# MikeWangWZHL/VidIL

Hardware: AMD Instinct MI355X
Metric: frames/sec whole-node (BLIP caption+filt + CLIP visual-token) 224^2 8f/video (higher is better)
Workload: dtype bf16

## Files before the change

vidil_amd/csrc/attention.hip:

```cpp
#include <type_traits>

#include "common.h"
#include "gemm_epilogue.h"

namespace {

template <typename T>
struct AttnP {
  const T* q;
  const T* k;
  const T* vt;
  T* out;
  const int32_t* kv_len;
  const int32_t* kv_index;
  const int32_t* group_start;
  int Bq, H, Nq, Nk, Tq_cap, Tk_cap, NP, kv_group, causal, causal_off, ldo, n_kv;
  int out_mode;
  int tiled;
  int rb;
  int ostage;
  const float* q32;
  long long ldq32;
  float q_scale;
};
// ... 94 lines not shown
#pragma unroll
  for (int r = 0; r < 16; ++r) {
    const float e = __builtin_amdgcn_exp2f(__builtin_fmaf(S[r], kLog2e, -mc));
    S[r] = e;
    ps += e;
  }
  l = FIRST ? ps : l + ps;
#pragma unroll
  for (int hb = 0; hb < 2; ++hb)
#pragma unroll
    for (int j = 0; j < 8; ++j) pf[hb][j] = (T)S[hb * 8 + j];
}

template <typename T, bool MASKED = true, bool LAZY = true, bool FIRST = false, typename VFrag>
__device__ __forceinline__ void softmax_pv_tile(f32x16& S, int key0, int klim, bool need_mask, float& m, float& l,
                                                f32x16 (&O)[2], VFrag&& vfrag) {
  typename Elt<T>::x8 pf[2];
  softmax_tile<T, MASKED, FIRST, LAZY>(S, key0, klim, need_mask, m, l, O, pf);
#pragma unroll
  for (int hb = 0; hb < 2; ++hb) {
#pragma unroll
    for (int dt = 0; dt < 2; ++dt) {
      const typename Elt<T>::x8 vf = vfrag(dt, hb);
      O[dt] = Elt<T>::mfma32(vf, pf[hb], O[dt]);
    }
  }
}

template <typename T, typename VFrag>
__device__ __forceinline__ void softmax_pv_tile_psplit(f32x16& S, int key0, int klim, bool need_mask, float& m, float& l,
                                                       f32x16 (&O)[2], VFrag&& vfrag) {
  const int hi = (threadIdx.x & 63) >> 5;
  if (need_mask) {
#pragma unroll
    for (int r = 0; r < 16; ++r) {
      const int key = key0 + (r & 3) + 8 * (r >> 2) + 4 * hi;
      if (key >= klim) S[r] = -INFINITY;
    }
  }
  float mt = S[0];
#pragma unroll
  for (int r = 1; r < 16; ++r) mt = fmaxf(mt, S[r]);
  mt = fmaxf(mt, __shfl_xor(mt, 32, 64));
  const float mn = fmaxf(m, mt);
  const float mc = (mn == -INFINITY ? 0.f : mn) * kLog2e;
  const float alpha = __builtin_amdgcn_exp2f(__builtin_fmaf(m, kLog2e, -mc));
  l *= alpha;
  m = mn;
#pragma unroll
  for (int dt = 0; dt < 2; ++dt)
#pragma unroll
    for (int r = 0; r < 16; ++r) O[dt][r] *= alpha;
  typename Elt<T>::x8 ph[2], pl[2];
  float ps = 0.f;
#pragma unroll
  for (int r = 0; r < 16; ++r) {
    const float e = __builtin_amdgcn_exp2f(__builtin_fmaf(S[r], kLog2e, -mc));
    ps += e;
    const T eh = Elt<T>::from_f32(e);
    ph[r >> 3][r & 7] = eh;
    pl[r >> 3][r & 7] = Elt<T>::from_f32(e - (float)eh);
  }
  l += ps;
#pragma unroll
  for (int hb = 0; hb < 2; ++hb) {
#pragma unroll
    for (int dt = 0; dt < 2; ++dt) {
      const typename Elt<T>::x8 vf = vfrag(dt, hb);
      O[dt] = Elt<T>::mfma32(vf, pl[hb], O[dt]);
      O[dt] = Elt<T>::mfma32(vf, ph[hb], O[dt]);
    }
  }
}

template <typename T>
__device__ __forceinline__ void store_rows(const AttnP<T>& p, const RowInfo& ri, int h, const f32x16 (&O)[2], float inv) {
  using f16x4 = typename Elt<T>::x4;
  using f16 = T;
  if (!ri.valid) return;
  const int hi = (threadIdx.x & 63) >> 5;
  if (p.out_mode >= 2) {
    const int pl = p.ldo / 3;
    f16* og = p.out + ((size_t)ri.qb * p.Nq + ri.t) * p.ldo + h * 64 + 4 * hi;
#pragma unroll
    for (int dt = 0; dt < 2; ++dt)
#pragma unroll
      for (int rq = 0; rq < 4; ++rq) {
        f16x4 vh, vl;
#pragma unroll
        for (int e = 0; e < 4; ++e) {
          const float v = O[dt][rq * 4 + e] * inv;
          vh[e] = Elt<T>::from_f32(v);
          vl[e] = Elt<T>::from_f32(v - (float)vh[e]);
        }
        *(f16x4*)(og + dt * 32 + rq * 8) = vh;
        *(f16x4*)(og + pl + dt * 32 + rq * 8) = vl;
        if (p.out_mode == 2) *(f16x4*)(og + 2 * pl + dt * 32 + rq * 8) = vh;
      }
    return;
  }
  if (p.out_mode == 1) {
    uint8_t* o8 = (uint8_t*)p.out + ((size_t)ri.qb * p.Nq + ri.t) * p.ldo + h * 64 + 4 * hi;
#pragma unroll
    for (int dt = 0; dt < 2; ++dt)
#pragma unroll
      for (int rq = 0; rq < 4; ++rq)
        *(uint32_t*)(o8 + dt * 32 + rq * 8) = pack4_fp8(O[dt][rq * 4 + 0] * inv, O[dt][rq * 4 + 1] * inv, O[dt][rq * 4 + 2] * inv,
                                                        O[dt][rq * 4 + 3] * inv);
    return;
  }
  f16* og = p.out + ((size_t)ri.qb * p.Nq + ri.t) * p.ldo + h * 64 + 4 * hi;
#pragma unroll
  for (int dt = 0; dt < 2; ++dt)
#pragma unroll
    for (int rq = 0; rq < 4; ++rq) {
      const f16x4 v = {(f16)(O[dt][rq * 4 + 0] * inv), (f16)(O[dt][rq * 4 + 1] * inv), (f16)(O[dt][rq * 4 + 2] * inv),
                       (f16)(O[dt][rq * 4 + 3] * inv)};
      *(f16x4*)(og + dt * 32 + rq * 8) = v;
    }
}

template <typename T>
__device__ __forceinline__ void store_rows_lds(const AttnP<T>& p, const RowInfo& ri, int h, const f32x16 (&O)[2], float inv, char* scratch) {
  using f16 = T;
  using f16x4 = typename Elt<T>::x4;
  using f16x8 = typename Elt<T>::x8;
  const int lane = threadIdx.x & 63;
  const int hi = lane >> 5, l31 = lane & 31;
  const long long own = ri.valid ? (long long)(((size_t)ri.qb * p.Nq + ri.t) * p.ldo + h * 64) : -1;
  long long dst[2];
#pragma unroll
  for (int i = 0; i < 2; ++i) {
    const int r = i * 16 + (lane >> 2);
    const int lo = __shfl((int)(own & 0xffffffffLL), r, 64), hi32 = __shfl((int)(own >> 32), r, 64);
    dst[i] = ((long long)hi32 << 32) | (unsigned int)lo;
  }
#pragma unroll
  for (int dt = 0; dt < 2; ++dt) {
#pragma unroll
    for (int rq = 0; rq < 4; ++rq) {
      const f16x4 v = {(f16)(O[dt][rq * 4 + 0] * inv), (f16)(O[dt][rq * 4 + 1] * inv), (f16)(O[dt][rq * 4 + 2] * inv),
                       (f16)(O[dt][rq * 4 + 3] * inv)};
      *(f16x4*)(scratch + l31 * 64 + ((rq ^ ((l31 >> 1) & 3)) << 4) + hi * 8) = v;
    }
#pragma unroll
    for (int i = 0; i < 2; ++i) {
      const int r = i * 16 + (lane >> 2), c = lane & 3;
      const f16x8 v = *(const f16x8*)(scratch + r * 64 + ((c ^ ((r >> 1) & 3)) << 4));
      if (dst[i] >= 0) *(f16x8*)(p.out + dst[i] + dt * 32 + c * 8) = v;
    }
  }
}

template <typename T, int NKT, int NW>
__global__ __launch_bounds__(NW * 64, NW == 8 ? 4 : 2) void attn_lds_kernel(const AttnP<T> p) {
  using f16 = T;
  using f16x8 = typename Elt<T>::x8;
  constexpr int NKEY = NKT * 32;
  constexpr int VROW = NKEY + 8;
  constexpr int NT = NW * 64;
  extern __shared__ __attribute__((aligned(16))) char smem[];
  f16* Ks = (f16*)smem;
  f16* Vs = (f16*)(smem + NKEY * KROW * 2);

  const int tid = threadIdx.x;
  const int lane = tid & 63;
  const int wave = __builtin_amdgcn_readfirstlane(tid >> 6);
  const int hi = lane >> 5, l31 = lane & 31;
  const int h = blockIdx.y;
  int bk, first, count;
  resolve_unit(p, blockIdx.z, bk, first, count);
  const int rows = count * p.Nq;
  const int nk = p.Nk;
  const int rows_per_wg = NW * 32 * (nk <= NKEY ? p.rb : 1);
  const int base = blockIdx.x * rows_per_wg;
  if (base >= rows) return;

  const f16* kg = p.k + ((size_t)bk * p.H + h) * p.Tk_cap * 64;
  const f16* vg = p.vt + ((size_t)bk * p.H + h) * 64 * (size_t)p.NP;
  constexpr int KIT = (NKEY * 8 + NT - 1) / NT;
  constexpr int VIT = (64 * NKT * 4 + NT - 1) / NT;
  auto stage = [&](int k0) {
    f16x8 kreg[KIT], vreg[VIT];
#pragma unroll
    for (int i = 0; i < KIT; ++i) {
      const int q = tid + i * NT;
      const int row = q >> 3, c = q & 7;
      kreg[i] = zero8<T>();
      if (q < NKEY * 8 && k0 + row < nk) kreg[i] = *(const f16x8*)(kg + (size_t)(k0 + row) * 64 + c * 8);
    }
    if (p.NP == 0) {
      const f16* vrow = p.vt + ((size_t)bk * p.H + h) * p.Tk_cap * 64;
#pragma unroll
      for (int i = 0; i < KIT; ++i) {
        const int q = tid + i * NT;
        const int c = q / NKEY, r = q - c * NKEY;
        vreg[i] = zero8<T>();
        if (q < NKEY * 8 && k0 + r < nk) vreg[i] = *(const f16x8*)(vrow + (size_t)(k0 + r) * 64 + c * 8);
      }
    } else {
#pragma unroll
      for (int i = 0; i < VIT; ++i) {
        const int q = tid + i * NT;
        const int d = q / (NKT * 4), kc = q - d * (NKT * 4);
        const int pos0 = k0 + kc * 8;
        vreg[i] = zero8<T>();
        if (q < 64 * NKT * 4 && (pos0 & ~15) < nk && pos0 + 8 <= p.NP) vreg[i] = *(const f16x8*)(vg + (size_t)d * p.NP + pos0);
      }
    }
#pragma unroll
    for (int i = 0; i < KIT; ++i) {
      const int q = tid + i * NT;
      if (q < NKEY * 8) *(f16x8*)(Ks + (q >> 3) * KROW + (q & 7) * 8) = kreg[i];
    }
    if (p.NP == 0) {
#pragma unroll
      for (int i = 0; i < KIT; ++i) {
        const int q = tid + i * NT;
        const int c = q / NKEY, r = q - c * NKEY;
        if (q < NKEY * 8) {
          const int col = vt_pos(r);
#pragma unroll
          for (int e = 0; e < 8; ++e) Vs[(c * 8 + e) * VROW + col] = vreg[i][e];
        }
      }
    } else {
#pragma unroll
      for (int i = 0; i < VIT; ++i) {
        const int q = tid + i * NT;
        const int d = q / (NKT * 4), kc = q - d * (NKT * 4);
        const int pos0 = k0 + kc * 8;
        if (q < 64 * NKT * 4) {
          f16x8 v = vreg[i];
          if ((pos0 | 15) + 1 > nk) {
#pragma unroll
            for (int e = 0; e < 8; ++e)
              if (vt_pos(pos0 + e) >= nk) v[e] = (f16)0.f;
          }
          *(f16x8*)(Vs + d * VROW + kc * 8) = v;
        }
      }
    }
  };

  auto stage_next = [&](int k0) {
    for (int q = tid; q < NKEY * 8; q += NT) {
      const int row = q >> 3, c = q & 7;
      f16x8 v = zero8<T>();
      if (k0 + row < nk) v = *(const f16x8*)(kg + (size_t)(k0 + row) * 64 + c * 8);
      *(f16x8*)(Ks + row * KROW + c * 8) = v;
    }
    if (p.NP == 0) {
      const f16* vrow = p.vt + ((size_t)bk * p.H + h) * p.Tk_cap * 64;
      for (int q = tid; q < NKEY * 8; q += NT) {
        const int c = q / NKEY, r = q - c * NKEY;
        f16x8 v = zero8<T>();
        if (k0 + r < nk) v = *(const f16x8*)(vrow + (size_t)(k0 + r) * 64 + c * 8);
        const int col = vt_pos(r);
#pragma unroll
        for (int e = 0; e < 8; ++e) Vs[(c * 8 + e) * VROW + col] = v[e];
      }
    }
    for (int q = tid; p.NP != 0 && q < 64 * NKT * 4; q += NT) {
      const int d = q / (NKT * 4), kc = q - d * (NKT * 4);
      const int pos0 = k0 + kc * 8;
      const int blk_end = (pos0 | 15) + 1;
      f16x8 v = zero8<T>();
      if (blk_end <= nk) {
        v = *(const f16x8*)(vg + (size_t)d * p.NP + pos0);
      } else if ((pos0 & ~15) < nk && pos0 + 8 <= p.NP) {
        v = *(const f16x8*)(vg + (size_t)d * p.NP + pos0);
#pragma unroll
        for (int e = 0; e < 8; ++e)
          if (vt_pos(pos0 + e) >= nk) v[e] = (f16)0.f;
      }
      *(f16x8*)(Vs + d * VROW + kc * 8) = v;
    }
  };

  const int nblk = nk <= NKEY ? p.rb : 1;
  RowInfo ri;
  f16x8 qf[4];
  bool active;
  auto load_q = [&](int rbi) {
    const int v0 = base + (rbi * NW + wave) * 32;
    active = v0 < rows;
    ri = row_info(p, (active ? v0 : 0) + l31, first, rows);
    const f16* qg = p.q + (((size_t)ri.qb * p.H + h) * p.Tq_cap + ri.t) * 64 + hi * 8;
#pragma unroll
    for (int ks = 0; ks < 4; ++ks) qf[ks] = *(const f16x8*)(qg + ks * 16);
  };
  load_q(0);
  stage(0);
  __syncthreads();
#pragma unroll 1
  for (int rbi = 0; rbi < nblk; ++rbi) {
    if (rbi > 0) {
      load_q(rbi);
      if (!active) break;
    }
    int kmin = ri.klim;
#pragma unroll
    for (int o = 32; o > 0; o >>= 1) {
      const int x = __shfl_xor(kmin, o, 64);
      kmin = x < kmin ? x : kmin;
    }

    float m = -INFINITY, l = 0.f;
    f32x16 O[2];
#pragma unroll
    for (int dt = 0; dt < 2; ++dt)
#pragma unroll
      for (int r = 0; r < 16; ++r) O[dt][r] = 0.f;

#pragma unroll 1
    for (int k0 = 0; k0 < nk; k0 += NKEY) {
      if (rbi == 0 && k0 > 0) {
        __syncthreads();
        stage_next(k0);
        __syncthreads();
      }
      if (!active) continue;

#pragma unroll 1
      for (int kt = 0; kt < NKT; ++kt) {
        if (k0 + kt * 32 >= nk) break;
        f32x16 S;
#pragma unroll
        for (int r = 0; r < 16; ++r) S[r] = 0.f;
#pragma unroll
        for (int ks = 0; ks < 4; ++ks) {
          const f16x8 kf = *(const f16x8*)(Ks + (kt * 32 + l31) * KROW + ks * 16 + hi * 8);
          S = Elt<T>::mfma32(kf, qf[ks], S);
        }
        const bool need_mask = (k0 + kt * 32 + 32) > kmin;
        auto vfrag = [&](int dt, int hb) { return *(const f16x8*)(Vs + (dt * 32 + l31) * VROW + (kt * 2 + hb) * 16 + 8 * hi); };
        if (need_mask) softmax_pv_tile<T, true>(S, k0 + kt * 32, ri.klim, true, m, l, O, vfrag);
        else softmax_pv_tile<T, false>(S, k0 + kt * 32, ri.klim, false, m, l, O, vfrag);
      }
    }
    if (!active) break;
    l += __shfl_xor(l, 32, 64);
    if (p.out_mode == 0 && p.ostage)
      store_rows_lds(p, ri, h, O, l > 0.f ? 1.0f / l : 0.f, smem + NKEY * KROW * 2 + 64 * VROW * 2 + wave * 2048);
    else
      store_rows(p, ri, h, O, l > 0.f ? 1.0f / l : 0.f);
  }
}

constexpr int LONG_NKT = 4;
constexpr int LONG_NKEY = LONG_NKT * 32;
constexpr int kLongMaxNk = 16384;

template <typename T, int NW>
__global__ __launch_bounds__(NW * 64, NW == 8 ? 4 : 2) void attn_long_kernel(const AttnP<T> p) {
  using f16 = T;
  using f16x8 = typename Elt<T>::x8;
  constexpr int NKT = LONG_NKT, NKEY = LONG_NKEY;
  constexpr int VROW = NKEY + 8;
  constexpr int NT = NW * 64;
  constexpr int BUF = NKEY * KROW * 2 + 64 * VROW * 2;
  constexpr int KIT = NKEY * 8 / NT;
  static_assert(NKEY * 8 % NT == 0 && 64 * NKT * 4 == NKEY * 8, "a chunk is a whole number of pieces per thread");
  extern __shared__ __attribute__((aligned(16))) char smem[];

  const int tid = threadIdx.x;
  const int lane = tid & 63;
  const int wave = __builtin_amdgcn_readfirstlane(tid >> 6);
  const int hi = lane >> 5, l31 = lane & 31;
  const int h = blockIdx.y;
  int bk, first, count;
  resolve_unit(p, blockIdx.z, bk, first, count);
  const int rows = count * p.Nq;
  const int nk = p.Nk;
  const int base = blockIdx.x * (NW * 32);
  if (base >= rows) return;

  const f16* kg = p.k + ((size_t)bk * p.H + h) * p.Tk_cap * 64;
  const f16* vg = p.vt + ((size_t)bk * p.H + h) * 64 * (size_t)p.NP;
  const f16* vrow = p.vt + ((size_t)bk * p.H + h) * p.Tk_cap * 64;
  const bool vrm = p.NP == 0;

  f16x8 kreg[KIT], vreg[KIT];
  const __amdgpu_buffer_rsrc_t rk = uniform_rsrc(kg, (uint32_t)nk * 128u);
  const __amdgpu_buffer_rsrc_t rv = vrm ? uniform_rsrc(vrow, (uint32_t)nk * 128u) : uniform_rsrc(vg, 128u * (uint32_t)p.NP);
  auto gload = [&](int k0) {
#pragma unroll
    for (int i = 0; i < KIT; ++i) {
      const int q = tid + i * NT;
      kreg[i] = __builtin_bit_cast(f16x8, __builtin_amdgcn_raw_buffer_load_b128(rk, (k0 * 8 + q) * 16, 0, 0));
    }
    if (vrm) {
#pragma unroll
      for (int i = 0; i < KIT; ++i) {
        const int q = tid + i * NT;
        const int c = q / NKEY, r = q - c * NKEY;
        vreg[i] = __builtin_bit_cast(f16x8, __builtin_amdgcn_raw_buffer_load_b128(rv, (k0 + r) * 128 + c * 16, 0, 0));
      }
    } else {
#pragma unroll
      for (int i = 0; i < KIT; ++i) {
        const int q = tid + i * NT;
        const int d = q / (NKT * 4), kc = q - d * (NKT * 4);
        const int pos0 = k0 + kc * 8;
        const bool in = (pos0 & ~15) < nk && pos0 + 8 <= p.NP;
        vreg[i] = __builtin_bit_cast(f16x8, __builtin_amdgcn_raw_buffer_load_b128(rv, in ? (d * p.NP + pos0) * 2 : (int)0x80000000, 0, 0));
      }
    }
  };
  auto lstore = [&](int k0, char* buf) {
    f16* Ks = (f16*)buf;
    f16* Vs = (f16*)(buf + NKEY * KROW * 2);
#pragma unroll
    for (int i = 0; i < KIT; ++i) {
      const int q = tid + i * NT;
      *(f16x8*)(Ks + (q >> 3) * KROW + (q & 7) * 8) = kreg[i];
    }
    if (vrm) {
#pragma unroll
      for (int i = 0; i < KIT; ++i) {
        const int q = tid + i * NT;
        const int c = q / NKEY, r = q - c * NKEY;
        const int col = vt_pos(r);
#pragma unroll
        for (int e = 0; e < 8; ++e) Vs[(c * 8 + e) * VROW + col] = vreg[i][e];
      }
    } else {
#pragma unroll
      for (int i = 0; i < KIT; ++i) {
        const int q = tid + i * NT;
        const int d = q / (NKT * 4), kc = q - d * (NKT * 4);
        const int pos0 = k0 + kc * 8;
        f16x8 v = vreg[i];
        if ((pos0 | 15) + 1 > nk) {
#pragma unroll
          for (int e = 0; e < 8; ++e)
            if (vt_pos(pos0 + e) >= nk) v[e] = (f16)0.f;
        }
        *(f16x8*)(Vs + d * VROW + kc * 8) = v;
      }
    }
  };

  const int v0 = base + wave * 32;
  const bool active = v0 < rows;
  const RowInfo ri = row_info(p, (active ? v0 : 0) + l31, first, rows);
  f16x8 qf[4];
  {
    const f16* qg = p.q + (((size_t)ri.qb * p.H + h) * p.Tq_cap + ri.t) * 64 + hi * 8;
#pragma unroll
    for (int ks = 0; ks < 4; ++ks) qf[ks] = *(const f16x8*)(qg + ks * 16);
  }
  gload(0);
  int kmin = ri.klim, kmax = ri.klim;
#pragma unroll
  for (int o = 32; o > 0; o >>= 1) {
    const int x = __shfl_xor(kmin, o, 64), y = __shfl_xor(kmax, o, 64);
    kmin = x < kmin ? x : kmin;
    kmax = y > kmax ? y : kmax;
  }
  float m = -INFINITY, l = 0.f;
  f32x16 O[2];
#pragma unroll
  for (int dt = 0; dt < 2; ++dt)
#pragma unroll
    for (int r = 0; r < 16; ++r) O[dt][r] = 0.f;

  lstore(0, smem);
  if (NKEY < nk) gload(NKEY);
  __syncthreads();
  int cur = 0;
#pragma unroll 1
  for (int k0 = 0; k0 < nk; k0 += NKEY) {
    if (active) {
      const f16* Ks = (const f16*)(smem + cur * BUF);
      const f16* Vs = (const f16*)(smem + cur * BUF + NKEY * KROW * 2);
#pragma unroll 1
      for (int kt = 0; kt < NKT; ++kt) {
        const int key0 = k0 + kt * 32;
        if (key0 >= nk || key0 >= kmax) break;
        f32x16 S;
#pragma unroll
        for (int r = 0; r < 16; ++r) S[r] = 0.f;
#pragma unroll
        for (int ks = 0; ks < 4; ++ks) {
          const f16x8 kf = *(const f16x8*)(Ks + (kt * 32 + l31) * KROW + ks * 16 + hi * 8);
          S = Elt<T>::mfma32(kf, qf[ks], S);
        }
        const bool need_mask = (key0 + 32) > kmin;
        auto vfrag = [&](int dt, int hb) { return *(const f16x8*)(Vs + (dt * 32 + l31) * VROW + (kt * 2 + hb) * 16 + 8 * hi); };
        if (need_mask) softmax_pv_tile<T, true>(S, key0, ri.klim, true, m, l, O, vfrag);
        else softmax_pv_tile<T, false>(S, key0, ri.klim, false, m, l, O, vfrag);
      }
    }
    if (k0 + NKEY < nk) {
      lstore(k0 + NKEY, smem + (cur ^ 1) * BUF);
      if (k0 + 2 * NKEY < nk) gload(k0 + 2 * NKEY);
    }
    __syncthreads();
    cur ^= 1;
  }
  if (!active) return;
  l += __shfl_xor(l, 32, 64);
  const float inv = l > 0.f ? 1.0f / l : 0.f;
  if (p.ostage) store_rows_lds(p, ri, h, O, inv, smem + wave * 2048);
  else store_rows(p, ri, h, O, inv);
}

typedef short s16x4 __attribute__((ext_vector_type(4)));

__device__ __forceinline__ void attn_glds16(const void* g, char* lds) {
  __builtin_amdgcn_global_load_lds((const __attribute__((address_space(1))) void*)g,
                                   (__attribute__((address_space(3))) void*)lds, 16, 0, 0);
}

template <typename T>
__device__ __forceinline__ void store_rows_stream(__amdgpu_buffer_rsrc_t rsrc, uint32_t row_off, const f32x16 (&O)[2], float inv,
                                                  char* scratch) {
  using f16 = T;
  using f16x4 = typename Elt<T>::x4;
  const int lane = threadIdx.x & 63;
  const int hi = lane >> 5, l31 = lane & 31;
  uint32_t dst[2];
#pragma unroll
  for (int i = 0; i < 2; ++i) dst[i] = (uint32_t)__shfl((int)row_off, i * 16 + (lane >> 2), 64);
#pragma unroll
  for (int dt = 0; dt < 2; ++dt) {
#pragma unroll
    for (int rq = 0; rq < 4; ++rq) {
      const f16x4 v = {(f16)(O[dt][rq * 4 + 0] * inv), (f16)(O[dt][rq * 4 + 1] * inv), (f16)(O[dt][rq * 4 + 2] * inv),
                       (f16)(O[dt][rq * 4 + 3] * inv)};
      *(f16x4*)(scratch + l31 * 64 + ((rq ^ ((l31 >> 1) & 3)) << 4) + hi * 8) = v;
    }
#pragma unroll
    for (int i = 0; i < 2; ++i) {
      const int r = i * 16 + (lane >> 2), c = lane & 3;
      const u32x4 v = *(const u32x4*)(scratch + r * 64 + ((c ^ ((r >> 1) & 3)) << 4));
      __builtin_amdgcn_raw_buffer_store_b128(v, rsrc, dst[i] + (uint32_t)((dt * 32 + c * 8) * 2), 0, 0);
    }
  }
}

__device__ __forceinline__ void store_rows_stream_fp8(__amdgpu_buffer_rsrc_t rsrc, uint32_t row_off, const f32x16 (&O)[2], float inv,
                                                      char* scratch) {
  const int lane = threadIdx.x & 63;
  const int hi = lane >> 5, l31 = lane & 31;
  uint32_t dst[2];
#pragma unroll
  for (int i = 0; i < 2; ++i) dst[i] = (uint32_t)__shfl((int)row_off, i * 16 + (lane >> 2), 64);
#pragma unroll
  for (int dt = 0; dt < 2; ++dt)
#pragma unroll
    for (int rq = 0; rq < 4; ++rq) {
      const int chunk = dt * 2 + (rq >> 1), in_chunk = (rq & 1) * 8 + hi * 4;
      *(uint32_t*)(scratch + l31 * 64 + ((chunk ^ ((l31 >> 1) & 3)) << 4) + in_chunk) =
          pack4_fp8(O[dt][rq * 4 + 0] * inv, O[dt][rq * 4 + 1] * inv, O[dt][rq * 4 + 2] * inv, O[dt][rq * 4 + 3] * inv);
    }
#pragma unroll
  for (int i = 0; i < 2; ++i) {
    const int r = i * 16 + (lane >> 2), c = lane & 3;
    const u32x4 v = *(const u32x4*)(scratch + r * 64 + ((c ^ ((r >> 1) & 3)) << 4));
    __builtin_amdgcn_raw_buffer_store_b128(v, rsrc, dst[i] + (uint32_t)(c * 16), 0, 0);
  }
}

template <typename T, int NKT, bool OUT8>
__global__ __launch_bounds__(512, 4) void attn_stream_kernel(const AttnP<T> p) {
  using f16x8 = typename Elt<T>::x8;
#ifndef VIDIL_ATTN_KA
#define VIDIL_ATTN_KA ((NKT + 1) / 2)
#endif
  constexpr int KA = VIDIL_ATTN_KA;
  constexpr int VSUB = 1152;
  constexpr int TILE = 4096 + 4 * VSUB;
  extern __shared__ __attribute__((aligned(16))) char smem[];
  const int tid = threadIdx.x;
  const int lane = tid & 63;
  const int wave = __builtin_amdgcn_readfirstlane(tid >> 6);
  const int nunits = p.n_kv * p.H;
  const int nk = p.Nk;
  const size_t kv_unit = (size_t)p.Tk_cap * 128;
  const int stride = gridDim.x;
  int u = blockIdx.x;
  if (u >= nunits) return;

  if (wave == 7) {
    auto issue_half = [&](int uu, int kt, int pc0) {
      const char* gb = (const char*)(pc0 == 0 ? p.k : p.vt) + (size_t)uu * kv_unit;
      char* dst = smem + kt * TILE;
#pragma unroll
      for (int pc = pc0; pc < pc0 + 4; ++pc) {
        int r, cb;
        if (pc < 4) {
          r = pc * 8 + (lane >> 3);
          cb = ((lane & 7) ^ ((r >> 1) & 7)) * 16;
        } else {
          r = lane >> 1;
          cb = (pc - 4) * 32 + (lane & 1) * 16;
        }
        int key = kt * 32 + r;
        key = key < nk - 1 ? key : nk - 1;
#if defined(VIDIL_ATTN_ABLATE) && (VIDIL_ATTN_ABLATE & 1)
        if (uu != (int)blockIdx.x) continue;
#endif
        attn_glds16(gb + (uint32_t)(key * 128 + cb), dst + (pc < 4 ? pc * 1024 : 4096 + (pc - 4) * VSUB));
      }
    };
    auto issue_first = [&](int uu) {
#pragma unroll
      for (int kt = 0; kt < KA; ++kt) issue_half(uu, kt, 0);
#pragma unroll
      for (int kt = 0; kt < KA - 1; ++kt) issue_half(uu, kt, 4);
    };
    auto issue_second = [&](int uu) {
#pragma unroll
      for (int kt = KA; kt < NKT; ++kt) issue_half(uu, kt, 0);
#pragma unroll
      for (int kt = KA - 1; kt < NKT; ++kt) issue_half(uu, kt, 4);
    };
    issue_first(u);
    for (;;) {
      asm volatile("s_waitcnt vmcnt(0)" ::: "memory");
      __builtin_amdgcn_s_barrier();
      issue_second(u);
      asm volatile("s_waitcnt vmcnt(0)" ::: "memory");
      __builtin_amdgcn_s_barrier();
      u += stride;
      if (u >= nunits) break;
      issue_first(u);
    }
    return;
  }

  const int hi = lane >> 5, l31 = lane & 31;
  const int sw = (l31 >> 1) & 7;
  const int row = wave * 32 + l31;
  const bool valid = row < p.Nq;
  const int vc = valid ? row : p.Nq - 1;
  const int vlane = ((lane >> 4) & 1) * VSUB + (hi * 4 + ((lane & 15) >> 2)) * 32 + (lane & 3) * 8;
  char* scratch = smem + NKT * TILE + wave * 2048;
  f16x8 qf[4];
  const uint32_t q_off = (uint32_t)(vc * 128 + hi * 16);
  const __amdgpu_buffer_rsrc_t rsrc_q = uniform_rsrc(p.q, (uint32_t)nunits * p.Tq_cap * 128);
  auto load_q = [&](int uu, f16x8 (&dst)[4]) {
    const uint32_t ub = (uint32_t)uu * p.Tq_cap * 128;
#pragma unroll
    for (int ks = 0; ks < 4; ++ks)
      dst[ks] = __builtin_bit_cast(f16x8, __builtin_amdgcn_raw_buffer_load_b128(rsrc_q, q_off + ks * 32, ub, 0));
  };
  const uint32_t row_off = valid ? (uint32_t)row * p.ldo * (OUT8 ? 1 : 2) : 0x80000000u;
  load_q(u, qf);
  asm volatile("" ::"v"(qf[0]), "v"(qf[1]), "v"(qf[2]), "v"(qf[3]));
  auto read_k2 = [&](int kt, int h2, f16x8 (&kf)[2]) {
    const char* ks_ = smem + kt * TILE + l31 * 128;
#pragma unroll
    for (int j = 0; j < 2; ++j) kf[j] = *(const f16x8*)(ks_ + ((((h2 * 2 + j) * 2 + hi) ^ sw) << 4));
  };
  auto read_v2 = [&](int kt, int hb, f16x8 (&vf)[2]) {
    const char* vs_ = smem + kt * TILE + 4096 + vlane + hb * 512;
#pragma unroll
    for (int dt = 0; dt < 2; ++dt) {
      const char* a = vs_ + dt * (2 * VSUB);
// ... 385 lines not shown
    }
    f16* const o = og + (qd >> 2) * 32 + (qd & 3) * 8;
    if (p.out_mode >= 2) {
      f16x4 vh, vl;
#pragma unroll
      for (int e = 0; e < 4; ++e) {
        const float v = acc[e] * inv;
        vh[e] = Elt<T>::from_f32(v);
        vl[e] = Elt<T>::from_f32(v - (float)vh[e]);
      }
      *(f16x4*)o = vh;
      *(f16x4*)(o + pl) = vl;
      *(f16x4*)(o + 2 * pl) = vh;
    } else {
      f16x4 v;
#pragma unroll
      for (int e = 0; e < 4; ++e) v[e] = (f16)(acc[e] * inv);
      *(f16x4*)o = v;
    }
  }
}

template <typename T, bool SPLIT>
__device__ __forceinline__ void store_rows_wave(const AttnP<T>& p, const RowInfo& ri, int h, const f32x16 (&O)[2], float inv, char* scratch) {
  using f16 = T;
  using f16x4 = typename Elt<T>::x4;
  using f16x8 = typename Elt<T>::x8;
  const int lane = threadIdx.x & 63;
  const int hi = lane >> 5, l31 = lane & 31;
  const int pl = p.ldo / 3;
  const long long own = ri.valid ? (long long)(((size_t)ri.qb * p.Nq + ri.t) * p.ldo + h * 64) : -1;
  long long dst[2];
#pragma unroll
  for (int i = 0; i < 2; ++i) {
    const int r = i * 16 + (lane >> 2);
    const int lo = __shfl((int)(own & 0xffffffffLL), r, 64), hi32 = __shfl((int)(own >> 32), r, 64);
    dst[i] = ((long long)hi32 << 32) | (unsigned int)lo;
  }
#pragma unroll
  for (int pass = 0; pass < (SPLIT ? 2 : 1); ++pass) {
#pragma unroll
    for (int dt = 0; dt < 2; ++dt) {
#pragma unroll
      for (int rq = 0; rq < 4; ++rq) {
        f16x4 v;
#pragma unroll
        for (int e = 0; e < 4; ++e) {
          const float o = O[dt][rq * 4 + e] * inv;
          const f16 oh = Elt<T>::from_f32(o);
          v[e] = pass == 0 ? oh : Elt<T>::from_f32(o - (float)oh);
        }
        *(f16x4*)(scratch + l31 * 64 + ((rq ^ ((l31 >> 1) & 3)) << 4) + hi * 8) = v;
      }
#pragma unroll
      for (int i = 0; i < 2; ++i) {
        const int r = i * 16 + (lane >> 2), c = lane & 3;
        const f16x8 v = *(const f16x8*)(scratch + r * 64 + ((c ^ ((r >> 1) & 3)) << 4));
        if (dst[i] >= 0) {
          f16* const og = p.out + dst[i] + dt * 32 + c * 8;
          if (!SPLIT) {
            *(f16x8*)og = v;
          } else if (pass == 0) {
            *(f16x8*)og = v;
            *(f16x8*)(og + 2 * pl) = v;
          } else {
            *(f16x8*)(og + pl) = v;
          }
        }
      }
    }
  }
}

template <typename T>
__global__ __launch_bounds__(256, 5) void attn_wave_kernel(const AttnP<T> p) {
  using f16 = T;
  using f16x8 = typename Elt<T>::x8;
  __shared__ __attribute__((aligned(16))) char ostage[4 * 2048];
  const int lane = threadIdx.x & 63;
  const int wave = __builtin_amdgcn_readfirstlane(threadIdx.x >> 6);
  const int hi = lane >> 5, l31 = lane & 31;
  const int u = blockIdx.x * 4 + wave;
  if (u >= p.H * p.n_kv) return;
  const int z = u / p.H, h = u - z * p.H;
  int bk, first, count;
  resolve_unit(p, z, bk, first, count);
  const int rows = count * p.Nq;
  if (rows <= 0) return;
  const int nk = p.Nk;
  const RowInfo ri = row_info(p, l31, first, rows);
  const f16* kg = p.k + ((size_t)bk * p.H + h) * p.Tk_cap * 64;
  const f16* vg = p.vt + ((size_t)bk * p.H + h) * 64 * (size_t)p.NP;
  const f16* qg = p.q + (((size_t)ri.qb * p.H + h) * p.Tq_cap + ri.t) * 64 + hi * 8;
  int krow = l31 < nk ? l31 : nk - 1;
  const f16* kr = kg + (size_t)krow * 64 + hi * 8;
  f16x8 kf[4], qf[4], vf[2][2];
#pragma unroll
  for (int ks = 0; ks < 4; ++ks) {
    kf[ks] = *(const f16x8*)(kr + ks * 16);
    qf[ks] = *(const f16x8*)(qg + ks * 16);
  }
#pragma unroll
  for (int dt = 0; dt < 2; ++dt)
#pragma unroll
    for (int hb = 0; hb < 2; ++hb) {
      const int blk0 = hb * 16;
      vf[dt][hb] = zero8<T>();
      if (blk0 < nk) vf[dt][hb] = *(const f16x8*)(vg + (size_t)(dt * 32 + l31) * p.NP + blk0 + 8 * hi);
    }
  f32x16 S;
#pragma unroll
  for (int r = 0; r < 16; ++r) S[r] = 0.f;
#pragma unroll
  for (int ks = 0; ks < 4; ++ks) S = Elt<T>::mfma32(kf[ks], qf[ks], S);
  float m = -INFINITY, l = 0.f;
  f32x16 O[2];
#pragma unroll
  for (int dt = 0; dt < 2; ++dt)
#pragma unroll
    for (int r = 0; r < 16; ++r) O[dt][r] = 0.f;
  softmax_pv_tile<T, true, true, true>(S, 0, ri.klim, true, m, l, O, [&](int dt, int hb) {
    const int blk0 = hb * 16;
    f16x8 v = vf[dt][hb];
#pragma unroll
    for (int e = 0; e < 8; ++e)
      if (blk0 + 4 * hi + (e & 3) + 8 * (e >> 2) >= nk) v[e] = (f16)0.f;
    return v;
  });
  l += __shfl_xor(l, 32, 64);
  const float inv = l > 0.f ? 1.0f / l : 0.f;
  __builtin_assume(p.out_mode != 1);
  if (!p.ostage) store_rows(p, ri, h, O, inv);
  else if (p.out_mode == 2) store_rows_wave<T, true>(p, ri, h, O, inv, ostage + wave * 2048);
  else store_rows_wave<T, false>(p, ri, h, O, inv, ostage + wave * 2048);
}

template <typename T, int NKT, int NW>
int launch_lds(const AttnP<T>& p, int max_rows, hipStream_t s) {
  constexpr int smem_kv = NKT * 32 * KROW * 2 + 64 * (NKT * 32 + 8) * 2;
  constexpr bool ostage = 2 * (smem_kv + NW * 2048) <= 160 * 1024;
  constexpr int smem = smem_kv + (ostage ? NW * 2048 : 0);
  static std::atomic<unsigned long long> attr_set{0};
  auto kern = attn_lds_kernel<T, NKT, NW>;
  if (const int rc_ = vidil_lds_opt_in(attr_set, (const void*)kern, smem, "attention")) return rc_;
  AttnP<T> q = p;
  q.ostage = (ostage && p.ldo % 8 == 0 && ((uintptr_t)p.out & 15) == 0) ? 1 : 0;
  q.rb = (p.Nk <= NKT * 32 && max_rows > NW * 32 && max_rows <= NW * 32 + NW * 16) ? 2 : 1;
  dim3 grid((max_rows + NW * 32 * q.rb - 1) / (NW * 32 * q.rb), p.H, p.n_kv);
  hipLaunchKernelGGL(kern, grid, dim3(NW * 64), smem, s, q);
  VIDIL_CHECK_LAUNCH("attention");
  return VIDIL_OK;
}

template <typename T>
bool stream_eligible(const AttnP<T>& p, int max_rows) {
  const char* e = vidil_dev_env("VIDIL_ATTN_STREAM");
  if (e != nullptr && e[0] == '0') return false;
  return p.NP == 0 && p.kv_len == nullptr && p.kv_index == nullptr && p.group_start == nullptr && p.kv_group == 1 && !p.causal &&
         max_rows > 128 && max_rows <= 224 && p.Nk > 192 && !p.tiled && (p.out_mode == 0 ? p.ldo % 8 == 0 : (p.out_mode == 1 && p.ldo % 16 == 0)) &&
         (uint64_t)p.Nq * p.ldo * 2 < 0x80000000ull && (uint64_t)p.n_kv * p.H * p.Tq_cap * 128 < 0x100000000ull && (((uintptr_t)p.k | (uintptr_t)p.vt | (uintptr_t)p.q | (uintptr_t)p.out) & 15) == 0;
}

template <typename T, int NKT>
int launch_stream(const AttnP<T>& p, hipStream_t s) {
  constexpr int smem = NKT * (4096 + 4 * 1152) + 8 * 2048;
  static_assert(2 * smem <= 160 * 1024, "two workgroups per CU");
  static std::atomic<unsigned long long> attr_set16{0}, attr_set8{0};
  const int n_cu = vidil_cu_count();
  auto kern16 = attn_stream_kernel<T, NKT, false>;
  auto kern8 = attn_stream_kernel<T, NKT, true>;
  if (const int rc_ = vidil_lds_opt_in(attr_set16, (const void*)kern16, smem, "attention (stream kernel)")) return rc_;
  if (const int rc_ = vidil_lds_opt_in(attr_set8, (const void*)kern8, smem, "attention (stream kernel)")) return rc_;
  AttnP<T> q = p;
  q.ostage = 1;
  const int units = p.n_kv * p.H, slots = 2 * n_cu;
  const int rounds = (units + slots - 1) / slots;
  const int grid = (units + rounds - 1) / rounds;
  if (p.out_mode == 1) hipLaunchKernelGGL(kern8, dim3(grid), dim3(512), smem, s, q);
  else hipLaunchKernelGGL(kern16, dim3(grid), dim3(512), smem, s, q);
  VIDIL_CHECK_LAUNCH("attention/stream");
  return VIDIL_OK;
}

template <typename T, int NW>
int launch_long(const AttnP<T>& p, int max_rows, hipStream_t s) {
  constexpr int smem = 2 * (LONG_NKEY * KROW * 2 + 64 * (LONG_NKEY + 8) * 2);
  static_assert(2 * smem <= 160 * 1024 && NW * 2048 <= smem, "two workgroups per CU; the output scratch fits the buffers");
  static std::atomic<unsigned long long> attr_set{0};
  auto kern = attn_long_kernel<T, NW>;
  if (const int rc_ = vidil_lds_opt_in(attr_set, (const void*)kern, smem, "attention (long-key kernel)")) return rc_;
  AttnP<T> q = p;
  q.ostage = (p.ldo % 8 == 0 && ((uintptr_t)p.out & 15) == 0) ? 1 : 0;
  q.rb = 1;
  dim3 grid((max_rows + NW * 32 - 1) / (NW * 32), p.H, p.n_kv);
  hipLaunchKernelGGL(kern, grid, dim3(NW * 64), smem, s, q);
  VIDIL_CHECK_LAUNCH("attention/long");
  return VIDIL_OK;
}

template <typename T, bool QS>
int launch_direct1(const AttnP<T>& p, hipStream_t s) {
  VIDIL_REQUIRE((long long)p.H * p.n_kv < 0x7fffffffLL, "attention: H=%d x %d kv batches overflow the unit index", p.H, p.n_kv);
  const int units = p.H * p.n_kv;
  const dim3 grid((units + 3) / 4);
  if (p.tiled) hipLaunchKernelGGL((attn_direct1_kernel<T, QS, 1, true>), grid, dim3(256), 0, s, p);
  else hipLaunchKernelGGL((attn_direct1_kernel<T, QS, 1, false>), grid, dim3(256), 0, s, p);
  VIDIL_CHECK_LAUNCH("attention/direct1");
  return VIDIL_OK;
}

template <typename T, int NW>
int launch_dsplit(const AttnP<T>& p, hipStream_t s) {
  VIDIL_REQUIRE((long long)p.H * p.n_kv < 0x7fffffffLL, "attention: H=%d x %d kv batches overflow the unit index", p.H, p.n_kv);
  constexpr int smem = NW * (8 * 64 * 16 + 2 * 64 * 4);
  static std::atomic<unsigned long long> attr_set{0};
  auto kern = attn_dsplit_kernel<T, NW>;
  if (const int rc_ = vidil_lds_opt_in(attr_set, (const void*)kern, smem, "attention (key-split kernel)")) return rc_;
  hipLaunchKernelGGL(kern, dim3(p.H * p.n_kv), dim3(NW * 64), smem, s, p);
  VIDIL_CHECK_LAUNCH("attention/dsplit");
  return VIDIL_OK;
}

template <typename T, int NKT>
int launch_any(const AttnP<T>& p, int max_rows, hipStream_t s) {
  if constexpr (NKT == 7)
    if (stream_eligible(p, max_rows)) return launch_stream<T, NKT>(p, s);
  if (max_rows <= 32 && NKT == 1 && !p.tiled) {
    VIDIL_REQUIRE((long long)p.H * p.n_kv < 0x7fffffffLL, "attention: H=%d x %d kv batches overflow the unit index", p.H, p.n_kv);
    AttnP<T> q = p;
    q.ostage = ((uintptr_t)p.out & 15) == 0 ? 1 : 0;
    hipLaunchKernelGGL(attn_wave_kernel<T>, dim3((p.H * p.n_kv + 3) / 4), dim3(256), 0, s, q);
    VIDIL_CHECK_LAUNCH("attention/wave");
    return VIDIL_OK;
  }
  if (max_rows <= 32) return launch_direct1<T, false>(p, s);
  if (max_rows > 128) return launch_lds<T, NKT, 8>(p, max_rows, s);
  return launch_lds<T, NKT, 4>(p, max_rows, s);
}

template <typename T>
int attention_dispatch(const AttnP<T>& p, int nkt, int max_rows, int Nk, bool key_split, hipStream_t s) {
  switch (nkt) {
    case 1: return launch_any<T, 1>(p, max_rows, s);
    case 2: return launch_any<T, 2>(p, max_rows, s);
    case 3: return launch_any<T, 3>(p, max_rows, s);
    case 4: return launch_any<T, 4>(p, max_rows, s);
    case 5: return launch_any<T, 5>(p, max_rows, s);
    case 6: return launch_any<T, 6>(p, max_rows, s);
    case 7: return launch_any<T, 7>(p, max_rows, s);
    case 8: return launch_any<T, 8>(p, max_rows, s);
    case 9: return launch_any<T, 9>(p, max_rows, s);
    default: break;
  }
  if (nkt <= 24) {
    if (max_rows <= 32) return launch_direct1<T, false>(p, s);
    if (max_rows > 128) return launch_lds<T, 7, 8>(p, max_rows, s);
    return launch_lds<T, 7, 4>(p, max_rows, s);
  }
  if (max_rows > 32 && !p.tiled && p.out_mode == 0 && Nk <= kLongMaxNk) {
    if (p.causal) {
      vidil_set_error("attention: causal masks are not supported by the long-key form (Nk=%d > 768)", Nk);
      return VIDIL_EUNSUP;
    }
    if (max_rows > 128) return launch_long<T, 8>(p, max_rows, s);
    return launch_long<T, 4>(p, max_rows, s);
  }
  if (key_split && p.tiled && max_rows <= 32 && p.out_mode != 1 && Nk <= kLongMaxNk) {
    if (p.causal) {
      vidil_set_error("attention: causal masks are not supported by the key-split form (Nk=%d > 768)", Nk);
      return VIDIL_EUNSUP;
    }
    return launch_dsplit<T, 4>(p, s);
  }
  vidil_set_error("attention: Nk=%d > 768 not supported by these kernels", Nk);
  return VIDIL_EUNSUP;
}

}

extern "C" int vidil_attention(const void* q, const void* k, const void* vt, void* out, const int32_t* kv_len,
                               const int32_t* kv_index, const int32_t* group_start, int32_t n_kv, int32_t max_group,
                               int32_t Bq, int32_t H, int32_t Nq, int32_t Nk, int32_t Tq_cap, int32_t Tk_cap, int32_t NP,
                               int32_t kv_group, int32_t causal, int32_t causal_off, int32_t ldo, int32_t kv_tiled,
                               int32_t dtype, int32_t out_dtype, void* stream) {
  VIDIL_REQUIRE(q && k && vt && out, "attention: null pointer");
  VIDIL_REQUIRE(Bq > 0 && H > 0 && Nq > 0 && Nk > 0, "attention: bad shape Bq=%d H=%d Nq=%d Nk=%d", Bq, H, Nq, Nk);
  VIDIL_REQUIRE(kv_tiled >= 0 && kv_tiled <= 2, "attention: kv_tiled=%d (0: rows, 1: fragment tiles, 2: fragment tiles, key-split form allowed)", kv_tiled);
  if (kv_tiled) {
    VIDIL_REQUIRE(Tq_cap >= Nq && Tk_cap >= Nk && Tk_cap % 32 == 0,
                  "attention: tiled K/V need Tk_cap=%d >= Nk=%d and a multiple of 32", Tk_cap, Nk);
    NP = Tk_cap;
  }
  VIDIL_REQUIRE(Tq_cap >= Nq && Tk_cap >= Nk && (NP == 0 || NP >= Nk), "attention: capacities too small");
  VIDIL_REQUIRE(NP % 16 == 0, "attention: NP=%d must be a multiple of 16 (V^T rows hold whole 16-key blocks)", NP);
  VIDIL_REQUIRE(ldo >= H * 64 && ldo % 8 == 0, "attention: ldo=%d must be >= H*64 and a multiple of 8", ldo);
  VIDIL_REQUIRE(kv_group > 0, "attention: kv_group=%d", kv_group);
  int units, max_rows;
  if (group_start != nullptr) {
    VIDIL_REQUIRE(kv_index == nullptr, "attention: group_start and kv_index are mutually exclusive");
    VIDIL_REQUIRE(n_kv > 0 && max_group > 0, "attention: group_start needs n_kv and max_group");
    units = n_kv;
    max_rows = max_group * Nq;
  } else if (kv_index != nullptr) {
    units = Bq;
    max_rows = Nq;
  } else {
    VIDIL_REQUIRE(Bq % kv_group == 0, "attention: Bq=%d not a multiple of kv_group=%d", Bq, kv_group);
    units = Bq / kv_group;
    max_rows = kv_group * Nq;
  }
  VIDIL_REQUIRE(H <= 65535 && units <= 65535, "attention: grid too large (H=%d units=%d)", H, units);
  const int nkt = (Nk + 31) / 32;
  VIDIL_REQUIRE(!kv_tiled || max_rows <= 32, "attention: tiled K/V serve at most 32 query rows per unit (got %d)", max_rows);
  VIDIL_REQUIRE(NP != 0 || max_rows > 32, "attention: row-major V (NP == 0) needs more than 32 query rows per unit (got %d)",
                max_rows);
  const bool split3 = out_dtype == (dtype | VIDIL_DT_SPLIT3);
  VIDIL_REQUIRE(out_dtype == dtype || split3 || (out_dtype == VIDIL_DT_FP8 && max_rows > 32 && ldo % 16 == 0),
                "attention: out_dtype=%d must equal dtype=%d (optionally | VIDIL_DT_SPLIT3), or be fp8 with more than 32 query "
                "rows per unit (staged kernel)", out_dtype, dtype);
  VIDIL_REQUIRE(!split3 || (ldo % 24 == 0 && ldo / 3 >= H * 64), "attention: split3 output needs ldo=%d = 3 planes of >= H*64, "
                "each a multiple of 8", ldo);
  VIDIL_DISPATCH_DTYPE(dtype, "attention", {
    const AttnP<T> p{(const T*)q, (const T*)k, (const T*)vt, (T*)out, kv_len, kv_index, group_start, Bq, H, Nq, Nk,
                     Tq_cap, Tk_cap, NP, kv_group, causal, causal_off, ldo, units, out_dtype == VIDIL_DT_FP8 ? 1 : (split3 ? 2 : 0),
                     kv_tiled ? 1 : 0, 1};
    return attention_dispatch<T>(p, nkt, max_rows, Nk, kv_tiled == 2, (hipStream_t)stream);
  });
}

namespace {

struct AttnF32P {
  const float* q;
  const float* k;
  const float* v;
  void* out;
  long long ldq, ldk, ldv, ldo;
  int q_off, k_off, v_off;
  int out_mode;
  int dtype16;
  const int32_t* kv_len;
  const int32_t* kv_index;
  const int32_t* group_start;
  int Bq, H, Nq, Nk, kv_rows, kv_group, causal, causal_off, n_kv;
  const int32_t* anc;
  int anc_ld, arena_rows;
  float scale;
  const float* rel_bias;
  int rel_bias_ld, rel_off;
};

template <typename T16>
__device__ __forceinline__ void store_f32_row(const AttnF32P& p, size_t row, int h, int d, float v) {
  if (p.out_mode == 0) {
    ((float*)p.out)[row * p.ldo + h * 64 + d] = v;
  } else {
    const long long pl = p.ldo / 3;
    T16* o = (T16*)p.out + row * p.ldo + h * 64 + d;
    const T16 hi = Elt<T16>::from_f32(v);
    const T16 lo = Elt<T16>::from_f32(v - (float)hi);
    o[0] = hi;
    o[pl] = lo;
    if (p.out_mode != 3) o[2 * pl] = hi;
  }
}

constexpr int F32_KC = 64;
constexpr int F32_LD = 68;
constexpr int F32_RB = 32;

template <typename T16>
__global__ __launch_bounds__(256) void attn_f32_kernel(const AttnF32P p) {
  __shared__ __attribute__((aligned(16))) float Ks[F32_KC * F32_LD];
  __shared__ __attribute__((aligned(16))) float Vs[F32_KC * F32_LD];
  __shared__ __attribute__((aligned(16))) float Qs[F32_RB * F32_LD];
  __shared__ __attribute__((aligned(16))) float Ps[4][4][F32_KC];
  const int tid = threadIdx.x, lane = tid & 63;
  const int wave = __builtin_amdgcn_readfirstlane(tid >> 6);
  const int h = blockIdx.y;
  int bk, first, count;
  resolve_unit(p, blockIdx.z, bk, first, count);
  const int rows = count * p.Nq;
  const int base = blockIdx.x * F32_RB;
  if (base >= rows) return;
  for (int i = tid; i < F32_RB * 16; i += 256) {
    const int r = i >> 4, c = i & 15;
    const RowInfo ri = row_info(p, base + r, first, rows);
    f32x4 qv = {0.f, 0.f, 0.f, 0.f};
// ... 673 lines not shown
```

Measured before the change: 5128.

## Add persistent warp-specialized attention kernel with producer waves prefetching K/V

```diff
diff --git a/vidil_amd/csrc/attention.hip b/vidil_amd/csrc/attention.hip
--- a/vidil_amd/csrc/attention.hip
+++ b/vidil_amd/csrc/attention.hip
@@ -270,6 +270,25 @@
   }
 }
 
+typedef short s16x4 __attribute__((ext_vector_type(4)));
+constexpr int vimg_pitch(int nkey) { return nkey * 32 + 128; }
+__device__ __forceinline__ void vimg_piece(int q, int pitch, int& r, int& c, int& off) {
+  const int blk = (q >> 3) & 3, c2 = q & 1;
+  r = (q >> 5) * 4 + ((q >> 1) & 3);
+  c = blk * 2 + c2;
+  off = blk * pitch + r * 32 + c2 * 16;
+}
+__device__ __forceinline__ int vimg_lane(int lane, int pitch) {
+  return ((lane >> 4) & 1) * pitch + ((lane >> 5) * 4 + ((lane & 15) >> 2)) * 32 + (lane & 3) * 8;
+}
+template <typename T>
+__device__ __forceinline__ typename Elt<T>::x8 vimg_frag(const char* a, int pitch, int dt, int step) {
+  const char* b = a + dt * 2 * pitch + step * 512;
+  const s16x4 lo = __builtin_amdgcn_ds_read_tr16_b64_v4i16((__attribute__((address_space(3))) s16x4*)(b));
+  const s16x4 hi4 = __builtin_amdgcn_ds_read_tr16_b64_v4i16((__attribute__((address_space(3))) s16x4*)(b + 256));
+  return __builtin_bit_cast(typename Elt<T>::x8, __builtin_shufflevector(lo, hi4, 0, 1, 2, 3, 4, 5, 6, 7));
+}
+
 template <typename T, int NKT, int NW>
 __global__ __launch_bounds__(NW * 64, NW == 8 ? 4 : 2) void attn_lds_kernel(const AttnP<T> p) {
   using f16 = T;
@@ -332,11 +351,16 @@
       if (q < NKEY * 8) *(f16x8*)(Ks + (q >> 3) * KROW + (q & 7) * 8) = kreg[i];
     }
     if (p.NP == 0) {
+#if defined(VIDIL_ATTN_LDS_ABLATE) && (VIDIL_ATTN_LDS_ABLATE & 1)
+      const bool tr_stores = p.ldo == -12345;
+#else
+      constexpr bool tr_stores = true;
+#endif
 #pragma unroll
       for (int i = 0; i < KIT; ++i) {
         const int q = tid + i * NT;
         const int c = q / NKEY, r = q - c * NKEY;
-        if (q < NKEY * 8) {
+        if (q < NKEY * 8 && tr_stores) {
           const int col = vt_pos(r);
 #pragma unroll
           for (int e = 0; e < 8; ++e) Vs[(c * 8 + e) * VROW + col] = vreg[i][e];
@@ -439,6 +463,9 @@
         __syncthreads();
       }
       if (!active) continue;
+#if defined(VIDIL_ATTN_LDS_ABLATE) && (VIDIL_ATTN_LDS_ABLATE & 4)
+      if (p.ldo != -12345) continue;
+#endif
 
 #pragma unroll 1
       for (int kt = 0; kt < NKT; ++kt) {
@@ -459,10 +486,164 @@
     }
     if (!active) break;
     l += __shfl_xor(l, 32, 64);
+#if defined(VIDIL_ATTN_LDS_ABLATE) && (VIDIL_ATTN_LDS_ABLATE & 2)
+    if (p.ldo != -12345) continue;
+#endif
     if (p.out_mode == 0 && p.ostage)
       store_rows_lds(p, ri, h, O, l > 0.f ? 1.0f / l : 0.f, smem + NKEY * KROW * 2 + 64 * VROW * 2 + wave * 2048);
     else
       store_rows(p, ri, h, O, l > 0.f ? 1.0f / l : 0.f);
+  }
+}
+
+constexpr int RES_LW = 3;
+constexpr int RES_CW = 8 - RES_LW;
+#ifndef VIDIL_ATTN_RESIDENT_PASSES
+#define VIDIL_ATTN_RESIDENT_PASSES 4
+#endif
+
+__device__ __forceinline__ void res_barrier() {
+  asm volatile("s_waitcnt lgkmcnt(0)" ::: "memory");
+  __builtin_amdgcn_s_barrier();
+  asm volatile("" ::: "memory");
+}
+
+template <typename T, int NKT>
+__global__ __launch_bounds__(512, 4) void attn_lds_resident_kernel(const AttnP<T> p, const int U) {
+  using f16 = T;
+  using f16x8 = typename Elt<T>::x8;
+  constexpr int NKEY = NKT * 32;
+  constexpr int VROW = NKEY + 8;
+  constexpr int VPITCH = vimg_pitch(NKEY);
+  constexpr int LT = RES_LW * 64;
+  constexpr int KIT = (NKEY * 8 + LT - 1) / LT;
+  extern __shared__ __attribute__((aligned(16))) char smem[];
+  f16* Ks = (f16*)smem;
+  char* Vs = smem + NKEY * KROW * 2;
+
+  const int tid = threadIdx.x;
+  const int lane = tid & 63;
+  const int wave = __builtin_amdgcn_readfirstlane(tid >> 6);
+  const int nk = p.Nk;
+  const int nunits = p.n_kv * p.H;
+  const int u0 = blockIdx.x * U;
+  const int n = nunits - u0 < U ? nunits - u0 : U;
+  if (n <= 0) return;
+
+  if (wave >= RES_CW) {
+    const int lt = tid - RES_CW * 64;
+    f16x8 kreg[KIT], vreg[KIT];
+    auto unit_rows = [&](int u) {
+      const int bk = u / p.H;
+      return (p.group_start[bk + 1] - p.group_start[bk]) * p.Nq;
+    };
+    int vr0, vc0, voff0;
+    vimg_piece(lt, VPITCH, vr0, vc0, voff0);
+    auto gload = [&](int u) {
+      const size_t ub = (size_t)u * p.Tk_cap * 128;
+      const __amdgpu_buffer_rsrc_t rk = uniform_rsrc((const char*)p.k + ub, (uint32_t)nk * 128u);
+      const __amdgpu_buffer_rsrc_t rv = uniform_rsrc((const char*)p.vt + ub, (uint32_t)nk * 128u);
+#pragma unroll
+      for (int i = 0; i < KIT; ++i)
+        kreg[i] = __builtin_bit_cast(f16x8, __builtin_amdgcn_raw_buffer_load_b128(rk, (lt + i * LT) * 16, 0, 0));
+#pragma unroll
+      for (int i = 0; i < KIT; ++i)
+        vreg[i] = __builtin_bit_cast(f16x8, __builtin_amdgcn_raw_buffer_load_b128(rv, (vr0 + i * (LT / 8)) * 128 + vc0 * 16, 0, 0));
+    };
+    auto lstore = [&]() {
+#pragma unroll
+      for (int i = 0; i < KIT; ++i) {
+        const int q = lt + i * LT;
+        if (q < NKEY * 8) *(f16x8*)(Ks + (q >> 3) * KROW + (q & 7) * 8) = kreg[i];
+      }
+#pragma unroll
+      for (int i = 0; i < KIT; ++i) {
+        const int q = lt + i * LT;
+        if (q < NKEY * 8) *(f16x8*)(Vs + voff0 + i * (LT / 8) * 32) = vreg[i];
+      }
+    };
+    bool has = unit_rows(u0) > 0;
+    if (has) gload(u0);
+#pragma unroll 1
+    for (int i = 0; i < n; ++i) {
+      res_barrier();
+      if (has) lstore();
+      res_barrier();
+      has = i + 1 < n && unit_rows(u0 + i + 1) > 0;
+      if (has) gload(u0 + i + 1);
+    }
+    return;
+  }
+
+  const int hi = lane >> 5, l31 = lane & 31;
+  const int vlane = vimg_lane(lane, VPITCH);
+  char* scratch = smem + NKEY * KROW * 2 + 64 * VROW * 2 + wave * 2048;
+  int qb_n = 0, t_n = 0, len_n = 0;
+  bool valid_n = false, act_n = false;
+  f16x8 qn[4];
+  auto prefetch = [&](int u) {
+    const int bk = u / p.H, h = u - bk * p.H;
+    const int first = p.group_start[bk];
+    const int rows = (p.group_start[bk + 1] - first) * p.Nq;
+    act_n = wave * 32 < rows;
+    if (!act_n) return;
+    const int v = wave * 32 + l31;
+    valid_n = v < rows;
+    const int vc = valid_n ? v : rows - 1;
+    const int g = vc / p.Nq;
+    qb_n = first + g;
+    t_n = vc - g * p.Nq;
+    len_n = p.kv_len != nullptr ? p.kv_len[qb_n] : nk;
+    const f16* qg = p.q + (((size_t)qb_n * p.H + h) * p.Tq_cap + t_n) * 64 + hi * 8;
+#pragma unroll
+    for (int ks = 0; ks < 4; ++ks) qn[ks] = *(const f16x8*)(qg + ks * 16);
+  };
+  prefetch(u0);
+#pragma unroll 1
+  for (int i = 0; i < n; ++i) {
+    const int u = u0 + i;
+    res_barrier();
+    const bool active = act_n;
+    RowInfo ri;
+    ri.qb = qb_n, ri.t = t_n, ri.valid = valid_n;
+    ri.klim = len_n < nk ? len_n : nk;
+    f16x8 qf[4];
+#pragma unroll
+    for (int ks = 0; ks < 4; ++ks) qf[ks] = qn[ks];
+    int kmin = ri.klim;
+#pragma unroll
+    for (int o = 32; o > 0; o >>= 1) {
+      const int x = __shfl_xor(kmin, o, 64);
+      kmin = x < kmin ? x : kmin;
+    }
+    res_barrier();
+    if (i + 1 < n) prefetch(u + 1);
+    if (!active) continue;
+
+    float m = -INFINITY, l = 0.f;
+    f32x16 O[2];
+#pragma unroll
+    for (int dt = 0; dt < 2; ++dt)
+#pragma unroll
+      for (int r = 0; r < 16; ++r) O[dt][r] = 0.f;
+#pragma unroll 1
+    for (int kt = 0; kt < NKT; ++kt) {
+      if (kt * 32 >= nk) break;
+      f32x16 S;
+#pragma unroll
+      for (int r = 0; r < 16; ++r) S[r] = 0.f;
+#pragma unroll
+      for (int ks = 0; ks < 4; ++ks) {
+        const f16x8 kf = *(const f16x8*)(Ks + (kt * 32 + l31) * KROW + ks * 16 + hi * 8);
+        S = Elt<T>::mfma32(kf, qf[ks], S);
+      }
+      const bool need_mask = (kt * 32 + 32) > kmin;
+      auto vfrag = [&](int dt, int hb) { return vimg_frag<T>(Vs + vlane, VPITCH, dt, kt * 2 + hb); };
+      if (need_mask) softmax_pv_tile<T, true>(S, kt * 32, ri.klim, true, m, l, O, vfrag);
+      else softmax_pv_tile<T, false>(S, kt * 32, ri.klim, false, m, l, O, vfrag);
+    }
+    l += __shfl_xor(l, 32, 64);
+    store_rows_lds(p, ri, u % p.H, O, l > 0.f ? 1.0f / l : 0.f, scratch);
   }
 }
 
@@ -625,7 +806,6 @@
   else store_rows(p, ri, h, O, inv);
 }
 
-typedef short s16x4 __attribute__((ext_vector_type(4)));
 
 __device__ __forceinline__ void attn_glds16(const void* g, char* lds) {
   __builtin_amdgcn_global_load_lds((const __attribute__((address_space(1))) void*)g,
@@ -1317,6 +1497,37 @@
   return VIDIL_OK;
 }
 
+template <typename T, int NKT>
+constexpr int resident_smem() { return NKT * 32 * KROW * 2 + 64 * (NKT * 32 + 8) * 2 + RES_CW * 2048; }
+
+template <typename T, int NKT>
+bool resident_eligible(const AttnP<T>& p, int max_rows) {
+  const char* e = vidil_dev_env("VIDIL_ATTN_RESIDENT");
+  if (e != nullptr && atoi(e) == 0) return false;
+  return p.group_start != nullptr && p.NP == 0 && !p.causal && !p.tiled && p.out_mode == 0 && p.ldo % 8 == 0 && max_rows > 32 &&
+         max_rows <= RES_CW * 32 && (long long)p.H * p.n_kv < 0x7fffffffLL &&
+         (((uintptr_t)p.k | (uintptr_t)p.vt | (uintptr_t)p.q | (uintptr_t)p.out) & 15) == 0;
+}
+
+template <typename T, int NKT>
+int launch_resident(const AttnP<T>& p, hipStream_t s) {
+  constexpr int smem = resident_smem<T, NKT>();
+  static std::atomic<unsigned long long> attr_set{0};
+  auto kern = attn_lds_resident_kernel<T, NKT>;
+  if (const int rc_ = vidil_lds_opt_in(attr_set, (const void*)kern, smem, "attention (resident kernel)")) return rc_;
+  const int units = p.n_kv * p.H, slots = 2 * vidil_cu_count();
+  const int rounds = (units + slots - 1) / slots;
+  int U = (rounds + VIDIL_ATTN_RESIDENT_PASSES - 1) / VIDIL_ATTN_RESIDENT_PASSES;
+  if (const char* e = vidil_dev_env("VIDIL_ATTN_RESIDENT"))
+    if (atoi(e) >= 2) U = atoi(e);
+  AttnP<T> q = p;
+  q.ostage = 1;
+  q.rb = 1;
+  hipLaunchKernelGGL(kern, dim3((units + U - 1) / U), dim3(512), smem, s, q, U);
+  VIDIL_CHECK_LAUNCH("attention/resident");
+  return VIDIL_OK;
+}
+
 template <typename T>
 bool stream_eligible(const AttnP<T>& p, int max_rows) {
   const char* e = vidil_dev_env("VIDIL_ATTN_STREAM");
@@ -1399,6 +1610,8 @@
     return VIDIL_OK;
   }
   if (max_rows <= 32) return launch_direct1<T, false>(p, s);
+  if constexpr (2 * resident_smem<T, NKT>() <= 160 * 1024)
+    if (resident_eligible<T, NKT>(p, max_rows)) return launch_resident<T, NKT>(p, s);
   if (max_rows > 128) return launch_lds<T, NKT, 8>(p, max_rows, s);
   return launch_lds<T, NKT, 4>(p, max_rows, s);
 }
```

Measured after the change: 5186 (median of 6 runs). 1.1% higher.
